# ubisoft/ubisoft-laforge-ZeroEGGS

Hardware: NVIDIA H100
Metric: frames/sec (train step, 60fps 75-joint pose) (higher is better)
Workload: dtype bf16

## Files before the change

ubisoft-laforge-zeroeggs_b200/csrc/decoder_bwd_tc.cu:

```cuda
#include "decoder_bwd_common.cuh"
#include "tc_dec_common.cuh"

namespace zeggs {

constexpr int BT_RING = 3;
constexpr int BT_XPART = 32768;
constexpr int BT_ACC_LD = 132;

struct BtGeom {
  int N2, N3, N4, P6;
  int kbH;
  int wslot;
  int slot_bytes;
  size_t off[4];
  size_t cta_bytes;
};

inline BtGeom make_btgeom(const DecGeom& g, const BwdGeom&) {
  BtGeom t;
  t.P6 = round_up(6 * g.U, 16); t.N2 = t.P6; t.N3 = t.P6 + 48; t.N4 = 16;
  t.kbH = ceil_div(g.H, 64);
  t.wslot = round_up(t.N3 * 128, 1024);
  t.slot_bytes = BT_XPART + 2 * t.wslot;
  size_t off = 0;
  t.off[0] = off; off += (size_t)t.kbH * t.N2 * 128;
  t.off[1] = off; off += (size_t)t.kbH * t.N3 * 128;
  t.off[2] = off; off += (size_t)t.kbH * t.N4 * 128;
  t.off[3] = off;
  t.cta_bytes = off;
  return t;
}

__global__ void pack_decoder_bwd_tc_kernel(DecGeom g, BtGeom tg, const float* __restrict__ Mfold, const float* __restrict__ W0,
                                           const float* __restrict__ Wih0, const float* __restrict__ Whh0,
                                           const float* __restrict__ Wih1, const float* __restrict__ Whh1, uint8_t* __restrict__ out) {
  const int H = g.H, U = g.U, A = g.A;
  const size_t per = tg.cta_bytes / 16, total = (size_t)g.G * per;
  for (size_t i = blockIdx.x * (size_t)blockDim.x + threadIdx.x; i < total; i += (size_t)gridDim.x * blockDim.x) {
    const int c = (int)(i / per);
    size_t ci = i % per;
    int chain = 2;
    for (int q = 0; q < 2; ++q) if (ci < tg.off[q + 1] / 16) { chain = q; break; }
    ci -= tg.off[chain] / 16;
    const int N = chain == 0 ? tg.N2 : chain == 1 ? tg.N3 : tg.N4;
    const int row = (int)(ci % N), cl = (int)((ci / N) % 8), kb = (int)(ci / ((size_t)8 * N));
    const int k0 = kb * 64 + cl * 8;
    const float* src = nullptr; size_t stride = 0;
    if (k0 < H) {
      if (chain <= 1 && row < 6 * U) {
        const int wsel = row / U, u = row % U, gq = wsel % 3, j = c * U + u;
        const size_t r = (size_t)(gq * H + k0);
        if (chain == 0) { src = (wsel < 3 ? Wih1 : Whh1) + r * H + j; stride = H; }
        else if (wsel < 3) { src = Wih0 + r * (A + H) + j; stride = A + H; }
        else { src = Whh0 + r * H + j; stride = H; }
      } else if (chain == 1 && row >= tg.P6) {
        const int rr = row - tg.P6, gq = rr / 16, lr = rr % 16;
        if (lr < U) { src = Mfold + ((size_t)(1 + gq) * H + k0) * H + c * U + lr; stride = H; }
        else if (lr >= 8 && lr < 11) { src = Wih0 + (size_t)(gq * H + k0) * (A + H) + H + P_OUT + (lr - 8); stride = A + H; }
      } else if (chain == 2) {
        if (row < U) { src = Mfold + (size_t)k0 * H + c * U + row; stride = H; }
        else if (row >= 8 && row < 11) { src = W0 + (size_t)k0 * A + P_OUT + (row - 8); stride = A; }
      }
    }
    __nv_bfloat16 t[8];
#pragma unroll
    for (int e = 0; e < 8; ++e) t[e] = __float2bfloat16_rn(src ? __ldg(src + (size_t)e * stride) : 0.f);
    uint8_t* dst = out + (size_t)c * tg.cta_bytes + tg.off[chain] + (size_t)kb * N * 128 + (size_t)row * 128 + (size_t)((cl ^ (row & 7)) << 4);
    *reinterpret_cast<uint4*>(dst) = *reinterpret_cast<const uint4*>(t);
  }
}

struct BtWs { uint8_t *g1img, *g0img, *dpaimg; const float* pre; float* dch; long long* dbg; size_t bytes; };
long long* tc_debug_buffer();
inline BtWs make_btws(void* base, const DecGeom& g) {
  BtWs w; size_t off = 0;
  auto take = [&](size_t n) { uint8_t* p = base ? (uint8_t*)base + off : nullptr; off += ((n + 1023) / 1024) * 1024; return p; };
  const size_t kbH = ceil_div(g.H, 64);
  w.g1img = take(kbH * 16384); w.g0img = take(kbH * 16384); w.dpaimg = take(kbH * 4096);
  w.pre = nullptr; w.dch = nullptr; w.dbg = nullptr;
  w.bytes = off; return w;
}

#define BTDBG1(ev) do { if (iw.dbg && c == 1 && lane == 0 && (T - 1 - t) < 64) iw.dbg[(T - 1 - t) * 32 + (ev)] = clock64(); } while (0)
#define BTDBG(ev) do { if (iw.dbg && c == 0 && lane == 0 && (T - 1 - t) < 64) iw.dbg[(T - 1 - t) * 32 + (ev)] = clock64(); } while (0)

template <int U>
__device__ __forceinline__ void store_img_row(uint8_t* img, int rows, int row, int j0, const float (&h)[U]) {
  __nv_bfloat16 t[U];
#pragma unroll
  for (int i = 0; i < U; ++i) t[i] = __float2bfloat16_rn(h[i]);
  uint8_t* p = img + img_off(rows, row, j0);
  if (U == 8) *reinterpret_cast<uint4*>(p) = *reinterpret_cast<const uint4*>(t);
  else *reinterpret_cast<uint2*>(p) = *reinterpret_cast<const uint2*>(t);
}

template <int U>
__global__ void __launch_bounds__(224, 1)
decoder_bwd_tc_kernel(zeggs_decoder_fwd_args a, DecGeom g, BwdGeom bg, BtGeom tg, DecWs w, BwdWs bw, BtWs iw, BwdArgsDev d,
                      const uint8_t* __restrict__ packed) {
  constexpr int P6 = (6 * U + 15) / 16 * 16, N2 = P6, N3 = P6 + 48, N4 = 16;
  constexpr int LD = BT_ACC_LD;
  extern __shared__ __align__(1024) uint8_t smem_raw[];
  uint8_t* smem = reinterpret_cast<uint8_t*>((reinterpret_cast<uintptr_t>(smem_raw) + 1023) & ~uintptr_t(1023));
  uint8_t* ring = smem;
  uint8_t* tail = ring + (size_t)BT_RING * tg.slot_bytes;
  uint64_t* full = reinterpret_cast<uint64_t*>(tail);
  uint64_t* empty = full + BT_RING;
  uint64_t* d_full = empty + BT_RING;
  float* accs = reinterpret_cast<float*>(tail + 512);
  float* c_w2r = accs + N3 * LD;
  float* c_gis = c_w2r + 6 * U;

  const int warp = __shfl_sync(0xffffffffu, (int)(threadIdx.x >> 5), 0), lane = threadIdx.x & 31;
  const int c = blockIdx.x, H = a.H, T = a.T;
  const int kbH = tg.kbH;
  const uint8_t* pk = packed + (size_t)c * tg.cta_bytes;
  constexpr int W_EPI = 4, W_PROD = 5, W_LOAD = 6;

  if (threadIdx.x == 0) {
    for (int i = 0; i < BT_RING; ++i) { mbar_init(&full[i], 2); mbar_init(&empty[i], 4); }
    for (int i = 0; i < 3; ++i) mbar_init(&d_full[i], 1);
    fence_mbar_init();
  }
  if (threadIdx.x < 6 * U) {
    const int n = threadIdx.x / U, u = threadIdx.x % U;
    c_w2r[threadIdx.x] = a.W2[(size_t)n * H + c * U + u] * a.out_std[n];
  }
  if (threadIdx.x < 3) c_gis[threadIdx.x] = 1.0f / a.in_std[P_OUT + threadIdx.x];
  __syncthreads();
  const size_t actH = (size_t)g.nbt * H * 32, act3 = (size_t)g.nbt * 3 * H * 32, act4 = (size_t)g.nbt * 4 * H * 32;

  if (warp == W_PROD) {
    if (lane == 0) {
      uint32_t it = 0;
      auto stream = [&](int chain, int nkb, int N, int kps) {
        const uint8_t* src = pk + tg.off[chain];
        const uint32_t tile = (uint32_t)N * 128;
        for (int kb = 0; kb < nkb; kb += kps, ++it) {
          const uint32_t s = it % BT_RING, ph = (it / BT_RING) & 1;
          const uint32_t bytes = (uint32_t)min(kps, nkb - kb) * tile;
          mbar_wait(&empty[s], ph ^ 1);
          mbar_arrive_expect_tx(&full[s], bytes);
          bulk_g2s(ring + (size_t)s * tg.slot_bytes + BT_XPART, src + (size_t)kb * tile, bytes, &full[s]);
        }
      };
      for (int t = T - 1; t >= 1; --t) {
        stream(0, kbH, tg.N2, 2); stream(1, kbH, tg.N3, 2);
        if (t > 1) stream(2, kbH, tg.N4, 8);
      }
    }
  } else if (warp == W_LOAD) {
    if (lane == 0) {
      uint32_t it = 0; unsigned epoch = 0;
      int t = T - 1; int sidx = 0;
      auto stream = [&](const uint8_t* img, int nkb, uint32_t tile_bytes) {
        grid_wait(bw.bar, (++epoch) * gridDim.x);
        if (iw.dbg && c == 0 && (T - 1 - t) < 64) iw.dbg[(T - 1 - t) * 32 + 2 * (sidx & 3)] = clock64();
        ++sidx;
        fence_proxy_async();
        const int kps = BT_XPART / (int)tile_bytes;
        for (int kb = 0; kb < nkb; kb += kps, ++it) {
          const uint32_t s = it % BT_RING, ph = (it / BT_RING) & 1;
          const uint32_t bytes = (uint32_t)min(kps, nkb - kb) * tile_bytes;
          mbar_wait(&empty[s], ph ^ 1);
          mbar_arrive_expect_tx(&full[s], bytes);
          bulk_g2s(ring + (size_t)s * tg.slot_bytes, img + (size_t)kb * tile_bytes, bytes, &full[s]);
        }
      };
      for (t = T - 1; t >= 1; --t) {
        sidx = 0;
        stream(iw.g1img, kbH, 16384); BTDBG(3);
        stream(iw.g0img, kbH, 16384); BTDBG(5);
        if (t > 1) { stream(iw.dpaimg, kbH, 4096); BTDBG(7); }
      }
    }
  } else if (warp < 4) {
    uint32_t it = 0;
    const uint64_t dR = make_smem_desc_sw128(ring);
    const uint32_t sstep = (uint32_t)(tg.slot_bytes >> 4);
    float d2[2][N2 / 2], d3[2][N3 / 2], d4[2][N4 / 2];
    auto chain_mma = [&](auto& dd, auto two, int nkb, int kps, uint32_t atile) {
      constexpr int N = 2 * (int)(sizeof(dd[0]) / sizeof(float));
      constexpr bool TWO = decltype(two)::value;
      const uint32_t astep = atile >> 4, wstep = (uint32_t)(N * 128) >> 4;
      uint32_t prev = 0;
      for (int kb = 0; kb < nkb; kb += kps, ++it) {
        const uint32_t s = it % BT_RING, ph = (it / BT_RING) & 1;
        const int nk = min(kps, nkb - kb);
        mbar_wait(&full[s], ph);
        uint64_t da = dR + (uint64_t)s * sstep, db = da + (BT_XPART >> 4);
        wgmma_fence();
        for (int kk = 0; kk < nk; ++kk, da += astep, db += wstep) {
#pragma unroll
          for (int ks = 0; ks < 4; ++ks) {
            const uint32_t acc = (kb + kk + ks) > 0 ? 1u : 0u;
            Wgmma<N>::mma(dd[0], da + 2 * ks, db + 2 * ks, acc);
            if constexpr (TWO) Wgmma<N>::mma(dd[1], da + 512 + 2 * ks, db + 2 * ks, acc);
          }
        }
        wgmma_commit();
        if (kb > 0) {
          wgmma_wait<1>();
          if (lane == 0) mbar_arrive(&empty[prev]);
        }
        prev = s;
      }
      wgmma_wait<0>();
      wgmma_fence_operands(dd[0]);
      if (TWO) wgmma_fence_operands(dd[1]);
      if (lane == 0) mbar_arrive(&empty[prev]);
      stage_acc<N>(dd[0], accs, LD, 0, TWO ? 64 : 32);
      if constexpr (TWO) stage_acc<N>(dd[1], accs, LD, 64, 64);
    };
    auto publish = [&](int i) {
      named_bar(1, 128);
      if (threadIdx.x == 0) mbar_arrive(&d_full[i]);
    };
    for (int t = T - 1; t >= 1; --t) {
      chain_mma(d2, std::true_type(), kbH, 2, 16384); publish(0); BTDBG(9);
      chain_mma(d3, std::true_type(), kbH, 2, 16384); publish(1); BTDBG(10);
      if (t > 1) { chain_mma(d4, std::false_type(), kbH, 8, 4096); publish(2); BTDBG(11); }
    }
  } else if (warp == W_EPI) {
    const int b = lane;
    const bool live = b < a.B;
    const int j0 = c * U;
    auto A = [&](int col, int blk) { return accs[(size_t)col * LD + 32 * blk + b]; };
    float dpq[7] = {0.f, 0.f, 0.f, 0.f, 0.f, 0.f, 0.f};
    float rpv[3] = {}, rqv[4] = {}, gpv[3] = {}, rq1v[4] = {}, ytv[6] = {}, e1p[3] = {}, e1q[4] = {}, e0p[3] = {}, e0q[4] = {};
    Q4 r_qinv, r_q1, r_E; V3 r_u, r_a1, r_a2, r_x; float r_k0 = 0.f, r_k1 = 0.f, r_k2 = 0.f;
    auto R_prefetch = [&](int t, bool have_dxp) {
      if (!live) return;
      const size_t bt = (size_t)b * T + t;
#pragma unroll
      for (int i = 0; i < 3; ++i) {
        rpv[i] = a.root_pos[bt * 3 + i];
        gpv[i] = have_dxp ? a.gaze_pos[(bt + 1) * 3 + i] : 0.f;
        e1p[i] = d.dRootPos ? d.dRootPos[(bt - 1) * 3 + i] : 0.f;
        e0p[i] = (!have_dxp && d.dRootPos) ? d.dRootPos[bt * 3 + i] : 0.f;
      }
#pragma unroll
      for (int i = 0; i < 4; ++i) {
        rqv[i] = a.root_rot[bt * 4 + i];
        rq1v[i] = a.root_rot[(bt - 1) * 4 + i];
        e1q[i] = d.dRootRot ? d.dRootRot[(bt - 1) * 4 + i] : 0.f;
        e0q[i] = (!have_dxp && d.dRootRot) ? d.dRootRot[bt * 4 + i] : 0.f;
      }
#pragma unroll
      for (int i = 0; i < 6; ++i) ytv[i] = a.Y[bt * P_OUT + i];
    };
    auto R_precompute = [&]() {
      if (!live) return;
      Q4 qt; qt.w = rqv[0]; qt.x = rqv[1]; qt.y = rqv[2]; qt.z = rqv[3];
      r_qinv = quat_inv(qt);
      r_u = v3(gpv[0] - rpv[0], gpv[1] - rpv[1], gpv[2] - rpv[2]);
      r_q1.w = rq1v[0]; r_q1.x = rq1v[1]; r_q1.y = rq1v[2]; r_q1.z = rq1v[3];
      r_a1 = a.dt * v3(ytv[0], ytv[1], ytv[2]);
      r_a2 = a.dt * v3(ytv[3], ytv[4], ytv[5]);
      const V3 wv = quat_mul_vec(r_q1, r_a2);
      r_E = quat_from_helical(wv);
      r_x = 0.5f * wv;
      const float a2 = dot(r_x, r_x), an = sqrtf(a2);
      if (an < 1e-5f) {
        const float rn = sqrtf(1.0f + a2), n = rn + 1e-5f;
        r_k0 = 1.0f / n; r_k1 = -1.0f / (n * n * rn); r_k2 = r_k1;
      } else {
        const float sn = sinf(an), cs = cosf(an);
        r_k0 = sn / an; r_k1 = -sn / an; r_k2 = (an * cs - sn) / (a2 * an);
      }
    };
    auto R_adjoint = [&](const float (&dgz)[3], bool have_dxp, float (&dch)[6]) {
#pragma unroll
      for (int i = 0; i < 6; ++i) dch[i] = 0.f;
      if (!live) return;
      V3 dp; Q4 dq;
      if (!have_dxp) {
        dp = v3(e0p[0], e0p[1], e0p[2]); dq.w = e0q[0]; dq.x = e0q[1]; dq.y = e0q[2]; dq.z = e0q[3];
      } else {
        dp = v3(dpq[0], dpq[1], dpq[2]); dq.w = dpq[3]; dq.x = dpq[4]; dq.y = dpq[5]; dq.z = dpq[6];
        Q4 dqc; V3 du;
        quat_mul_vec_bwd(r_qinv, r_u, v3(dgz[0], dgz[1], dgz[2]), dqc, du);
        dq.w += dqc.w; dq.x -= dqc.x; dq.y -= dqc.y; dq.z -= dqc.z;
        dp = dp - du;
      }
      Q4 dq_a, dq_b, dq_c, dE; V3 da1, da2;
      quat_mul_vec_bwd(r_q1, r_a1, dp, dq_a, da1);
      quat_mul_bwd(r_E, r_q1, dq, dE, dq_b);
      const V3 dEv = v3(dE.x, dE.y, dE.z);
      const V3 dw = 0.5f * (r_k0 * dEv + (r_k1 * dE.w + r_k2 * dot(dEv, r_x)) * r_x);
      quat_mul_vec_bwd(r_q1, r_a2, dw, dq_c, da2);
      dch[0] = a.dt * da1.x; dch[1] = a.dt * da1.y; dch[2] = a.dt * da1.z; dch[3] = a.dt * da2.x; dch[4] = a.dt * da2.y; dch[5] = a.dt * da2.z;
      dpq[0] = dp.x + e1p[0]; dpq[1] = dp.y + e1p[1]; dpq[2] = dp.z + e1p[2];
      dpq[3] = dq_a.w + dq_b.w + dq_c.w + e1q[0]; dpq[4] = dq_a.x + dq_b.x + dq_c.x + e1q[1];
      dpq[5] = dq_a.y + dq_b.y + dq_c.y + e1q[2]; dpq[6] = dq_a.z + dq_b.z + dq_c.z + e1q[3];
    };
    float dhz1[U], dhz0[U], dsum[16];
    float g1r[U], g1z[U], g1n[U], g1hn[U], g1hp[U], g1acc[U], prev[U];
    auto G1_prefetch = [&](int t) {
      const float* G = w.G1 + t * act4;
#pragma unroll
      for (int u = 0; u < U; ++u) {
        const int j = j0 + u;
        g1r[u] = G[(size_t)(0 * H + j) * 32 + b]; g1z[u] = G[(size_t)(1 * H + j) * 32 + b];
        g1n[u] = G[(size_t)(2 * H + j) * 32 + b]; g1hn[u] = G[(size_t)(3 * H + j) * 32 + b];
        g1hp[u] = w.H1[(t - 1) * actH + (size_t)j * 32 + b];
        g1acc[u] = t == T - 1 ? 0.f : bw.DH1[(size_t)j * 32 + b];
      }
      const float* P = iw.pre + ((size_t)(live ? b : 0) * T + t) * H + j0;
#pragma unroll
      for (int u4 = 0; u4 < U; u4 += 4) {
        const float4 v4 = live ? __ldg(reinterpret_cast<const float4*>(P + u4)) : make_float4(0.f, 0.f, 0.f, 0.f);
        prev[u4] = v4.x; prev[u4 + 1] = v4.y; prev[u4 + 2] = v4.z; prev[u4 + 3] = v4.w;
      }
    };
    auto G1_adjoint = [&](int t, const float (&fold)[U], const float (&dch)[6]) {
      float pr[U], pz[U], pn[U], pnr[U];
#pragma unroll
      for (int u = 0; u < U; ++u) {
        float dh = prev[u] + fold[u] + g1acc[u];
#pragma unroll
        for (int n = 0; n < 6; ++n) dh = fmaf(c_w2r[n * U + u], dch[n], dh);
        float dgi[3], dgh[3];
        gru_gate_bwd(dh, g1r[u], g1z[u], g1n[u], g1hn[u], g1hp[u], dgi, dgh, dhz1[u]);
        pr[u] = dgi[0]; pz[u] = dgi[1]; pn[u] = dgi[2]; pnr[u] = dgh[2];
      }
      store_img_row<U>(iw.g1img, 128, 0 * 32 + b, j0, pr); store_img_row<U>(iw.g1img, 128, 1 * 32 + b, j0, pz);
      store_img_row<U>(iw.g1img, 128, 2 * 32 + b, j0, pn); store_img_row<U>(iw.g1img, 128, 3 * 32 + b, j0, pnr);
      grid_arrive(bw.bar);
#pragma unroll
      for (int u = 0; u < U; ++u) {
        const int j = j0 + u;
        bw.DGI1[t * act3 + (size_t)(0 * H + j) * 32 + b] = pr[u]; bw.DGI1[t * act3 + (size_t)(1 * H + j) * 32 + b] = pz[u];
        bw.DGI1[t * act3 + (size_t)(2 * H + j) * 32 + b] = pn[u];
        bw.DGH1[t * act3 + (size_t)(0 * H + j) * 32 + b] = pr[u]; bw.DGH1[t * act3 + (size_t)(1 * H + j) * 32 + b] = pz[u];
        bw.DGH1[t * act3 + (size_t)(2 * H + j) * 32 + b] = pnr[u];
      }
      if (c == 0 && live) {
        float* dc = iw.dch + ((size_t)t * 32 + b) * 8;
#pragma unroll
        for (int n = 0; n < 6; ++n) dc[n] = dch[n];
      }
    };

    {
      const float zero3[3] = {0.f, 0.f, 0.f};
      float zeroU[U], dch[6];
#pragma unroll
      for (int u = 0; u < U; ++u) zeroU[u] = 0.f;
      R_prefetch(T - 1, false); R_precompute(); G1_prefetch(T - 1);
      R_adjoint(zero3, false, dch);
      G1_adjoint(T - 1, zeroU, dch);
    }
    for (int t = T - 1; t >= 1; --t) {
      const uint32_t ph = (uint32_t)((T - 1 - t) & 1);
      float gr[U], gz[U], gn[U], ghn[U], hp[U], acc[U];
      {
        const float* G = w.G0 + t * act4;
#pragma unroll
        for (int u = 0; u < U; ++u) {
          const int j = j0 + u;
          gr[u] = G[(size_t)(0 * H + j) * 32 + b]; gz[u] = G[(size_t)(1 * H + j) * 32 + b];
          gn[u] = G[(size_t)(2 * H + j) * 32 + b]; ghn[u] = G[(size_t)(3 * H + j) * 32 + b];
          hp[u] = w.H0[(t - 1) * actH + (size_t)j * 32 + b];
          acc[u] = t == T - 1 ? 0.f : bw.DH0[(size_t)j * 32 + b];
        }
      }
      mbar_wait(&d_full[0], ph);
      BTDBG(14);
      {
        float pr[U], pz[U], pn[U], pnr[U], dh1n[U];
#pragma unroll
        for (int u = 0; u < U; ++u) {
          const float oa = (A(0 * U + u, 0) + A(1 * U + u, 1)) + A(2 * U + u, 2);
          const float ob = (A(3 * U + u, 0) + A(4 * U + u, 1)) + A(5 * U + u, 3);
          float dgi[3], dgh[3];
          gru_gate_bwd(oa + acc[u], gr[u], gz[u], gn[u], ghn[u], hp[u], dgi, dgh, dhz0[u]);
          pr[u] = dgi[0]; pz[u] = dgi[1]; pn[u] = dgi[2]; pnr[u] = dgh[2];
          dh1n[u] = ob + dhz1[u];
        }
        store_img_row<U>(iw.g0img, 128, 0 * 32 + b, j0, pr); store_img_row<U>(iw.g0img, 128, 1 * 32 + b, j0, pz);
        store_img_row<U>(iw.g0img, 128, 2 * 32 + b, j0, pn); store_img_row<U>(iw.g0img, 128, 3 * 32 + b, j0, pnr);
        BTDBG(16);
        grid_arrive(bw.bar);
#pragma unroll
        for (int u = 0; u < U; ++u) bw.DH1[(size_t)(j0 + u) * 32 + b] = dh1n[u];
#pragma unroll
        for (int u = 0; u < U; ++u) {
          const int j = j0 + u;
          bw.DGI0[t * act3 + (size_t)(0 * H + j) * 32 + b] = pr[u]; bw.DGI0[t * act3 + (size_t)(1 * H + j) * 32 + b] = pz[u];
          bw.DGI0[t * act3 + (size_t)(2 * H + j) * 32 + b] = pn[u];
          bw.DGH0[t * act3 + (size_t)(0 * H + j) * 32 + b] = pr[u]; bw.DGH0[t * act3 + (size_t)(1 * H + j) * 32 + b] = pz[u];
          bw.DGH0[t * act3 + (size_t)(2 * H + j) * 32 + b] = pnr[u];
        }
      }
      float av[U];
#pragma unroll
      for (int u = 0; u < U; ++u) av[u] = w.A[t * actH + (size_t)(j0 + u) * 32 + b];
      mbar_wait(&d_full[1], ph);
      BTDBG(17);
      {
        float dpa[U], dh0n[U];
#pragma unroll
        for (int u = 0; u < U; ++u) {
          const float da = (A(0 * U + u, 0) + A(1 * U + u, 1)) + A(2 * U + u, 2);
          const float ob = (A(3 * U + u, 0) + A(4 * U + u, 1)) + A(5 * U + u, 3);
          dpa[u] = da * (av[u] > 0.f ? 1.f : av[u] + 1.f);
          dh0n[u] = ob + dhz0[u];
        }
#pragma unroll
        for (int r = 0; r < 16; ++r)
          dsum[r] = (A(P6 + r, 0) + A(P6 + 16 + r, 1)) + A(P6 + 32 + r, 2);
        store_img_row<U>(iw.dpaimg, 32, b, j0, dpa);
        BTDBG(18);
        if (t > 1) grid_arrive(bw.bar);
#pragma unroll
        for (int u = 0; u < U; ++u) { bw.DH0[(size_t)(j0 + u) * 32 + b] = dh0n[u]; bw.DPA[t * actH + (size_t)(j0 + u) * 32 + b] = dpa[u]; }
      }
      if (t == 1) break;
      R_prefetch(t - 1, true); R_precompute(); G1_prefetch(t - 1);
      mbar_wait(&d_full[2], ph);
      BTDBG(19);
      float tot[16];
#pragma unroll
      for (int r = 0; r < 16; ++r) tot[r] = A(r, 0) + dsum[r];
      float fold[U], dgz[3], dch[6];
#pragma unroll
      for (int u = 0; u < U; ++u) fold[u] = tot[u];
#pragma unroll
      for (int i = 0; i < 3; ++i) dgz[i] = tot[8 + i] * c_gis[i];
      R_adjoint(dgz, true, dch);
      BTDBG(20);
      G1_adjoint(t - 1, fold, dch);
    }
  }
}

__global__ void dy_scale_bf16_kernel(const float* __restrict__ dY, const float* __restrict__ os, size_t rows, int ld, __nv_bfloat16* __restrict__ out) {
  const size_t total = rows * (size_t)ld;
  for (size_t i = blockIdx.x * (size_t)blockDim.x + threadIdx.x; i < total; i += (size_t)gridDim.x * blockDim.x) {
    const size_t r = i / ld; const int n = (int)(i % ld);
    out[i] = __float2bfloat16_rn((dY && n < P_OUT) ? dY[r * P_OUT + n] * os[n] : 0.f);
  }
}

extern "C" size_t zeggs_decoder_packed_bwd_tc_bytes(int H, int S, int Z) {
  if (!tc_hidden_ok(H)) return 0;
  DecGeom g = make_geom(1, H, S, Z);
  BtGeom tg = make_btgeom(g, make_bgeom(g));
  return (size_t)g.G * tg.cta_bytes;
}
extern "C" size_t zeggs_decoder_bwd_tc_workspace_bytes(int H, int S, int Z) {
  if (!tc_hidden_ok(H)) return 0;
  return make_btws(nullptr, make_geom(1, H, S, Z)).bytes;
}
extern "C" int zeggs_decoder_pack_weights_bwd_tc(const zeggs_decoder_fwd_args* a, void* packed, void* stream_) {
  CtxScope ctx_scope(a ? a->ctx : nullptr);
  ZCHECK_ARG(a && packed, "decoder bwd tc pack: bad arguments");
  ZCHECK_SUPPORTED(tc_hidden_ok(a->H), "decoder bwd tc pack: hidden size %d unsupported (needs H %% 128 == 0, 384 <= H <= 1024)", a->H);
  const float* mfold = decoder_tc_mfold(*a);
  ZCHECK_ARG(mfold != nullptr, "decoder bwd tc pack: the forward pack (zeggs_decoder_pack_weights_tc -> args.packed_tc) must run first");
  DecGeom g = make_geom(a->B, a->H, a->S, a->Z);
  BwdGeom bg = make_bgeom(g);
  BtGeom tg = make_btgeom(g, bg);
  ZCHECK_ARG(g.U <= 8, "decoder bwd tc: unsupported units per CTA");
  ScopedTimer tm_pack("weight_pack", (cudaStream_t)stream_);
  pack_decoder_bwd_tc_kernel<<<592, 256, 0, (cudaStream_t)stream_>>>(g, tg, mfold, a->W0, a->W_ih0, a->W_hh0, a->W_ih1, a->W_hh1, (uint8_t*)packed);
  count_launch();
  ZCHECK_LAUNCH();
  return ZEGGS_OK;
}

template <int U>
static int launch_bt(const zeggs_decoder_fwd_args& a, const DecGeom& g, const BwdGeom& bg, const BtGeom& tg, const DecWs& w,
                     const BwdWs& bw, const BtWs& iw, const BwdArgsDev& d, const uint8_t* packed, cudaStream_t stream) {
  const size_t smem = 1024 + (size_t)BT_RING * tg.slot_bytes + 512 + (size_t)(tg.N3 * BT_ACC_LD + 6 * U + 16) * sizeof(float);
  static size_t checked_smem = 0;
  if (checked_smem != smem) {
    ZCHECK_CUDA(cudaFuncSetAttribute(decoder_bwd_tc_kernel<U>, cudaFuncAttributeMaxDynamicSharedMemorySize, (int)smem));
    int dev = 0, nsm = 0, occ = 0;
    ZCHECK_CUDA(cudaGetDevice(&dev));
    ZCHECK_CUDA(cudaDeviceGetAttribute(&nsm, cudaDevAttrMultiProcessorCount, dev));
    ZCHECK_CUDA(cudaOccupancyMaxActiveBlocksPerMultiprocessor(&occ, decoder_bwd_tc_kernel<U>, 224, smem));
    ZCHECK_ARG(occ * nsm >= g.G, "decoder bwd tc: cooperative grid of %d CTAs does not fit", g.G);
    checked_smem = smem;
  }
  void* args[] = {(void*)&a, (void*)&g, (void*)&bg, (void*)&tg, (void*)&w, (void*)&bw, (void*)&iw, (void*)&d, (void*)&packed};
  ZCHECK_CUDA(cudaLaunchCooperativeKernel((void*)decoder_bwd_tc_kernel<U>, dim3(g.G), dim3(224), args, smem, stream));
  count_launch();
  return ZEGGS_OK;
}

int decoder_bwd_tc_run(const zeggs_decoder_fwd_args& a, const zeggs_decoder_bwd_args& b, const DecGeom& g, const DecWs& w,
                       const BwdWs& bw, cudaStream_t stream) {
  BwdGeom bg = make_bgeom(g);
  ZCHECK_ARG(g.nbt == 1, "decoder bwd tc engine needs B <= 32 (got B=%d)", a.B);
  ZCHECK_ARG(b.packed_bwd_tc && b.workspace_tc, "decoder bwd tc: packed_bwd_tc / workspace_tc missing");
  BtGeom tg = make_btgeom(g, bg);
  ZCHECK_ARG((tg.kbH % 2) == 0, "decoder bwd tc: unsupported geometry");
  BtWs iw = make_btws(b.workspace_tc, g);
  iw.dbg = tc_debug_buffer();
  iw.dch = bw.DCH;
  const int H = a.H, ld = round_up(P_OUT, 8);
  const size_t rows = (size_t)a.B * a.T;
  char* p = scratch_base();
  ZCHECK_ARG(p != nullptr, "decoder bwd tc: scratch buffer missing (zeggs_ctx.scratch)");
  auto take = [&](size_t bytes) { char* r = p; p += (bytes + 255) / 256 * 256; return r; };
  __nv_bfloat16* dys = (__nv_bfloat16*)take(rows * ld * 2);
  __nv_bfloat16* w2t = (__nv_bfloat16*)take((size_t)H * ld * 2);
  float* pre = (float*)take(rows * H * sizeof(float));
  ZCHECK_ARG((size_t)(p - scratch_base()) <= scratch_bytes(), "decoder bwd tc: scratch buffer too small (%zu bytes needed)", (size_t)(p - scratch_base()));
  dy_scale_bf16_kernel<<<1184, 256, 0, stream>>>(b.dY, a.out_std, rows, ld, dys); count_launch();
  int rc = split_t_launch(a.W2, P_OUT, H, H, w2t, nullptr, ld, stream); if (rc) return rc;
  rc = tc_gemm_launch((int)rows, H, ld, dys, nullptr, ld, w2t, nullptr, ld, nullptr, pre, H, 0, 0, stream); if (rc) return rc;
  iw.pre = pre;
  BwdArgsDev d; d.dY = b.dY; d.dRootPos = b.dRootPos; d.dRootRot = b.dRootRot; d.packed = nullptr;
  return g.U == 4 ? launch_bt<4>(a, g, bg, tg, w, bw, iw, d, (const uint8_t*)b.packed_bwd_tc, stream)
                  : launch_bt<8>(a, g, bg, tg, w, bw, iw, d, (const uint8_t*)b.packed_bwd_tc, stream);
}

}
```

ubisoft-laforge-zeroeggs_b200/csrc/tc_common.cuh:

```cuda
#pragma once
#include <cuda.h>
#include <cuda_runtime.h>
#include <stdint.h>
#include <type_traits>

namespace zeggs {

__device__ __forceinline__ uint32_t smem_u32(const void* p) { return (uint32_t)__cvta_generic_to_shared(p); }

__device__ __forceinline__ void mbar_init(uint64_t* bar, uint32_t count) {
  asm volatile("mbarrier.init.shared::cta.b64 [%0], %1;\n" ::"r"(smem_u32(bar)), "r"(count) : "memory");
}
__device__ __forceinline__ void fence_mbar_init() {
  asm volatile("fence.mbarrier_init.release.cluster;\n" ::: "memory");
  asm volatile("fence.proxy.async.shared::cta;\n" ::: "memory");
}
__device__ __forceinline__ void mbar_arrive_expect_tx(uint64_t* bar, uint32_t bytes) {
  asm volatile("mbarrier.arrive.expect_tx.shared::cta.b64 _, [%0], %1;\n" ::"r"(smem_u32(bar)), "r"(bytes) : "memory");
}
__device__ __forceinline__ void mbar_arrive(uint64_t* bar) {
  asm volatile("mbarrier.arrive.shared::cta.b64 _, [%0];\n" ::"r"(smem_u32(bar)) : "memory");
}
__device__ __forceinline__ void mbar_wait(uint64_t* bar, uint32_t parity) {
  const uint32_t addr = smem_u32(bar);
  uint32_t done = 0;
#pragma unroll 1
  for (uint32_t it = 0; it < 20000000u; ++it) {
    asm volatile("{\n .reg .pred p;\n mbarrier.try_wait.parity.shared::cta.b64 p, [%1], %2;\n selp.u32 %0, 1, 0, p;\n}\n"
                 : "=r"(done) : "r"(addr), "r"(parity) : "memory");
    if (done) return;
  }
  __trap();
}

__device__ __forceinline__ bool elect_one_sync() {
  uint32_t pred;
  asm volatile("{\n .reg .pred p;\n elect.sync _|p, 0xffffffff;\n selp.u32 %0, 1, 0, p;\n}\n" : "=r"(pred));
  return pred != 0;
}

__device__ __forceinline__ void tma_prefetch_desc(const CUtensorMap* m) {
  asm volatile("prefetch.tensormap [%0];\n" ::"l"(reinterpret_cast<uint64_t>(m)) : "memory");
}
__device__ __forceinline__ void tma_load_2d(void* smem_dst, const CUtensorMap* m, uint64_t* bar, int c0, int c1) {
  asm volatile("cp.async.bulk.tensor.2d.shared::cluster.global.mbarrier::complete_tx::bytes [%0], [%1, {%3, %4}], [%2];\n"
               ::"r"(smem_u32(smem_dst)), "l"(reinterpret_cast<uint64_t>(m)), "r"(smem_u32(bar)), "r"(c0), "r"(c1) : "memory");
}
__device__ __forceinline__ void tma_load_3d(void* smem_dst, const CUtensorMap* m, uint64_t* bar, int c0, int c1, int c2) {
  asm volatile("cp.async.bulk.tensor.3d.shared::cluster.global.mbarrier::complete_tx::bytes [%0], [%1, {%3, %4, %5}], [%2];\n"
               ::"r"(smem_u32(smem_dst)), "l"(reinterpret_cast<uint64_t>(m)), "r"(smem_u32(bar)), "r"(c0), "r"(c1), "r"(c2) : "memory");
}

__device__ __forceinline__ void wgmma_fence() { asm volatile("wgmma.fence.sync.aligned;\n" ::: "memory"); }
__device__ __forceinline__ void wgmma_commit() { asm volatile("wgmma.commit_group.sync.aligned;\n" ::: "memory"); }
template <int n>
__device__ __forceinline__ void wgmma_wait() { asm volatile("wgmma.wait_group.sync.aligned %0;\n" ::"n"(n) : "memory"); }
template <int R>
__device__ __forceinline__ void wgmma_fence_operands(float (&d)[R]) {
#pragma unroll
  for (int i = 0; i < R; ++i) asm volatile("" : "+f"(d[i])::"memory");
}
__device__ __forceinline__ void named_bar(int id, int nthreads) { asm volatile("bar.sync %0, %1;\n" ::"r"(id), "r"(nthreads) : "memory"); }

template <int N> struct Wgmma;
template <> struct Wgmma<16> {
  static __device__ __forceinline__ void mma(float (&d)[8], uint64_t a, uint64_t b, uint32_t scale_d) {
    asm volatile("{\n .reg .pred p;\n setp.ne.b32 p, %10, 0;\n"
                 "wgmma.mma_async.sync.aligned.m64n16k16.f32.bf16.bf16 {%0, %1, %2, %3, %4, %5, %6, %7}, %8, %9, p, 1, 1, 0, 0;\n}\n"
                 : "+f"(d[0]), "+f"(d[1]), "+f"(d[2]), "+f"(d[3]), "+f"(d[4]), "+f"(d[5]), "+f"(d[6]), "+f"(d[7])
                 : "l"(a), "l"(b), "r"(scale_d));
  }
};
template <> struct Wgmma<24> {
  static __device__ __forceinline__ void mma(float (&d)[12], uint64_t a, uint64_t b, uint32_t scale_d) {
    asm volatile("{\n .reg .pred p;\n setp.ne.b32 p, %14, 0;\n"
                 "wgmma.mma_async.sync.aligned.m64n24k16.f32.bf16.bf16 {%0, %1, %2, %3, %4, %5, %6, %7, %8, %9, %10, %11}, %12, %13, p, 1, 1, 0, 0;\n}\n"
                 : "+f"(d[0]), "+f"(d[1]), "+f"(d[2]), "+f"(d[3]), "+f"(d[4]), "+f"(d[5]), "+f"(d[6]), "+f"(d[7]), "+f"(d[8]), "+f"(d[9]), "+f"(d[10]), "+f"(d[11])
                 : "l"(a), "l"(b), "r"(scale_d));
  }
};
template <> struct Wgmma<32> {
  static __device__ __forceinline__ void mma(float (&d)[16], uint64_t a, uint64_t b, uint32_t scale_d) {
    asm volatile("{\n .reg .pred p;\n setp.ne.b32 p, %18, 0;\n"
                 "wgmma.mma_async.sync.aligned.m64n32k16.f32.bf16.bf16 {%0, %1, %2, %3, %4, %5, %6, %7, %8, %9, %10, %11, %12, %13, %14, %15}, %16, %17, p, 1, 1, 0, 0;\n}\n"
                 : "+f"(d[0]), "+f"(d[1]), "+f"(d[2]), "+f"(d[3]), "+f"(d[4]), "+f"(d[5]), "+f"(d[6]), "+f"(d[7]), "+f"(d[8]), "+f"(d[9]), "+f"(d[10]), "+f"(d[11]), "+f"(d[12]), "+f"(d[13]), "+f"(d[14]), "+f"(d[15])
                 : "l"(a), "l"(b), "r"(scale_d));
  }
};
template <> struct Wgmma<40> {
  static __device__ __forceinline__ void mma(float (&d)[20], uint64_t a, uint64_t b, uint32_t scale_d) {
    asm volatile("{\n .reg .pred p;\n setp.ne.b32 p, %22, 0;\n"
                 "wgmma.mma_async.sync.aligned.m64n40k16.f32.bf16.bf16 {%0, %1, %2, %3, %4, %5, %6, %7, %8, %9, %10, %11, %12, %13, %14, %15, %16, %17, %18, %19}, %20, %21, p, 1, 1, 0, 0;\n}\n"
                 : "+f"(d[0]), "+f"(d[1]), "+f"(d[2]), "+f"(d[3]), "+f"(d[4]), "+f"(d[5]), "+f"(d[6]), "+f"(d[7]), "+f"(d[8]), "+f"(d[9]), "+f"(d[10]), "+f"(d[11]), "+f"(d[12]), "+f"(d[13]), "+f"(d[14]), "+f"(d[15]), "+f"(d[16]), "+f"(d[17]), "+f"(d[18]), "+f"(d[19])
                 : "l"(a), "l"(b), "r"(scale_d));
  }
};
template <> struct Wgmma<48> {
  static __device__ __forceinline__ void mma(float (&d)[24], uint64_t a, uint64_t b, uint32_t scale_d) {
    asm volatile("{\n .reg .pred p;\n setp.ne.b32 p, %26, 0;\n"
                 "wgmma.mma_async.sync.aligned.m64n48k16.f32.bf16.bf16 {%0, %1, %2, %3, %4, %5, %6, %7, %8, %9, %10, %11, %12, %13, %14, %15, %16, %17, %18, %19, %20, %21, %22, %23}, %24, %25, p, 1, 1, 0, 0;\n}\n"
                 : "+f"(d[0]), "+f"(d[1]), "+f"(d[2]), "+f"(d[3]), "+f"(d[4]), "+f"(d[5]), "+f"(d[6]), "+f"(d[7]), "+f"(d[8]), "+f"(d[9]), "+f"(d[10]), "+f"(d[11]), "+f"(d[12]), "+f"(d[13]), "+f"(d[14]), "+f"(d[15]), "+f"(d[16]), "+f"(d[17]), "+f"(d[18]), "+f"(d[19]), "+f"(d[20]), "+f"(d[21]), "+f"(d[22]), "+f"(d[23])
                 : "l"(a), "l"(b), "r"(scale_d));
  }
};
template <> struct Wgmma<80> {
  static __device__ __forceinline__ void mma(float (&d)[40], uint64_t a, uint64_t b, uint32_t scale_d) {
    asm volatile("{\n .reg .pred p;\n setp.ne.b32 p, %42, 0;\n"
                 "wgmma.mma_async.sync.aligned.m64n80k16.f32.bf16.bf16 {%0, %1, %2, %3, %4, %5, %6, %7, %8, %9, %10, %11, %12, %13, %14, %15, %16, %17, %18, %19, %20, %21, %22, %23, %24, %25, %26, %27, %28, %29, %30, %31, %32, %33, %34, %35, %36, %37, %38, %39}, %40, %41, p, 1, 1, 0, 0;\n}\n"
                 : "+f"(d[0]), "+f"(d[1]), "+f"(d[2]), "+f"(d[3]), "+f"(d[4]), "+f"(d[5]), "+f"(d[6]), "+f"(d[7]), "+f"(d[8]), "+f"(d[9]), "+f"(d[10]), "+f"(d[11]), "+f"(d[12]), "+f"(d[13]), "+f"(d[14]), "+f"(d[15]), "+f"(d[16]), "+f"(d[17]), "+f"(d[18]), "+f"(d[19]), "+f"(d[20]), "+f"(d[21]), "+f"(d[22]), "+f"(d[23]), "+f"(d[24]), "+f"(d[25]), "+f"(d[26]), "+f"(d[27]), "+f"(d[28]), "+f"(d[29]), "+f"(d[30]), "+f"(d[31]), "+f"(d[32]), "+f"(d[33]), "+f"(d[34]), "+f"(d[35]), "+f"(d[36]), "+f"(d[37]), "+f"(d[38]), "+f"(d[39])
                 : "l"(a), "l"(b), "r"(scale_d));
  }
};
template <> struct Wgmma<96> {
  static __device__ __forceinline__ void mma(float (&d)[48], uint64_t a, uint64_t b, uint32_t scale_d) {
    asm volatile("{\n .reg .pred p;\n setp.ne.b32 p, %50, 0;\n"
                 "wgmma.mma_async.sync.aligned.m64n96k16.f32.bf16.bf16 {%0, %1, %2, %3, %4, %5, %6, %7, %8, %9, %10, %11, %12, %13, %14, %15, %16, %17, %18, %19, %20, %21, %22, %23, %24, %25, %26, %27, %28, %29, %30, %31, %32, %33, %34, %35, %36, %37, %38, %39, %40, %41, %42, %43, %44, %45, %46, %47}, %48, %49, p, 1, 1, 0, 0;\n}\n"
                 : "+f"(d[0]), "+f"(d[1]), "+f"(d[2]), "+f"(d[3]), "+f"(d[4]), "+f"(d[5]), "+f"(d[6]), "+f"(d[7]), "+f"(d[8]), "+f"(d[9]), "+f"(d[10]), "+f"(d[11]), "+f"(d[12]), "+f"(d[13]), "+f"(d[14]), "+f"(d[15]), "+f"(d[16]), "+f"(d[17]), "+f"(d[18]), "+f"(d[19]), "+f"(d[20]), "+f"(d[21]), "+f"(d[22]), "+f"(d[23]), "+f"(d[24]), "+f"(d[25]), "+f"(d[26]), "+f"(d[27]), "+f"(d[28]), "+f"(d[29]), "+f"(d[30]), "+f"(d[31]), "+f"(d[32]), "+f"(d[33]), "+f"(d[34]), "+f"(d[35]), "+f"(d[36]), "+f"(d[37]), "+f"(d[38]), "+f"(d[39]), "+f"(d[40]), "+f"(d[41]), "+f"(d[42]), "+f"(d[43]), "+f"(d[44]), "+f"(d[45]), "+f"(d[46]), "+f"(d[47])
                 : "l"(a), "l"(b), "r"(scale_d));
  }
};
template <> struct Wgmma<128> {
  static __device__ __forceinline__ void mma(float (&d)[64], uint64_t a, uint64_t b, uint32_t scale_d) {
    asm volatile("{\n .reg .pred p;\n setp.ne.b32 p, %66, 0;\n"
                 "wgmma.mma_async.sync.aligned.m64n128k16.f32.bf16.bf16 {%0, %1, %2, %3, %4, %5, %6, %7, %8, %9, %10, %11, %12, %13, %14, %15, %16, %17, %18, %19, %20, %21, %22, %23, %24, %25, %26, %27, %28, %29, %30, %31, %32, %33, %34, %35, %36, %37, %38, %39, %40, %41, %42, %43, %44, %45, %46, %47, %48, %49, %50, %51, %52, %53, %54, %55, %56, %57, %58, %59, %60, %61, %62, %63}, %64, %65, p, 1, 1, 0, 0;\n}\n"
                 : "+f"(d[0]), "+f"(d[1]), "+f"(d[2]), "+f"(d[3]), "+f"(d[4]), "+f"(d[5]), "+f"(d[6]), "+f"(d[7]), "+f"(d[8]), "+f"(d[9]), "+f"(d[10]), "+f"(d[11]), "+f"(d[12]), "+f"(d[13]), "+f"(d[14]), "+f"(d[15]), "+f"(d[16]), "+f"(d[17]), "+f"(d[18]), "+f"(d[19]), "+f"(d[20]), "+f"(d[21]), "+f"(d[22]), "+f"(d[23]), "+f"(d[24]), "+f"(d[25]), "+f"(d[26]), "+f"(d[27]), "+f"(d[28]), "+f"(d[29]), "+f"(d[30]), "+f"(d[31]), "+f"(d[32]), "+f"(d[33]), "+f"(d[34]), "+f"(d[35]), "+f"(d[36]), "+f"(d[37]), "+f"(d[38]), "+f"(d[39]), "+f"(d[40]), "+f"(d[41]), "+f"(d[42]), "+f"(d[43]), "+f"(d[44]), "+f"(d[45]), "+f"(d[46]), "+f"(d[47]), "+f"(d[48]), "+f"(d[49]), "+f"(d[50]), "+f"(d[51]), "+f"(d[52]), "+f"(d[53]), "+f"(d[54]), "+f"(d[55]), "+f"(d[56]), "+f"(d[57]), "+f"(d[58]), "+f"(d[59]), "+f"(d[60]), "+f"(d[61]), "+f"(d[62]), "+f"(d[63])
                 : "l"(a), "l"(b), "r"(scale_d));
  }
};

__device__ __forceinline__ uint64_t make_smem_desc_sw128(const void* tile) {
  const uint32_t addr = smem_u32(tile);
  uint64_t d = 0;
  d |= (uint64_t)((addr & 0x3FFFFu) >> 4);
  d |= (uint64_t)1 << 16;
  d |= (uint64_t)(1024 >> 4) << 32;
  d |= (uint64_t)1 << 62;
  return d;
}

typedef CUresult (*PFN_encodeTiled)(CUtensorMap*, CUtensorMapDataType, cuuint32_t, void*, const cuuint64_t*,
                                    const cuuint64_t*, const cuuint32_t*, const cuuint32_t*, CUtensorMapInterleave,
                                    CUtensorMapSwizzle, CUtensorMapL2promotion, CUtensorMapFloatOOBfill);
inline PFN_encodeTiled get_encode_fn() {
  static PFN_encodeTiled fn = nullptr;
  if (!fn) {
    void* p = nullptr;
    cudaDriverEntryPointQueryResult q;
    if (cudaGetDriverEntryPoint("cuTensorMapEncodeTiled", &p, cudaEnableDefault, &q) == cudaSuccess &&
        q == cudaDriverEntryPointSuccess)
      fn = (PFN_encodeTiled)p;
  }
  return fn;
}

}
```

ubisoft-laforge-zeroeggs_b200/csrc/tc_dec_common.cuh:

```cuda
#pragma once
#include "decoder_common.cuh"
#include "tc_common.cuh"

namespace zeggs {

__host__ __device__ inline size_t img_off(int rows, int row, int k) {
  const int kb = k >> 6, c = (k & 63) >> 3, e = k & 7;
  return (size_t)kb * rows * 128 + (size_t)row * 128 + (size_t)((c ^ (row & 7)) << 4) + (size_t)e * 2;
}


__device__ __forceinline__ void bulk_g2s(void* smem_dst, const void* gsrc, uint32_t bytes, uint64_t* bar) {
  asm volatile("cp.async.bulk.shared::cluster.global.mbarrier::complete_tx::bytes [%0], [%1], %2, [%3];\n"
               ::"r"(smem_u32(smem_dst)), "l"(gsrc), "r"(bytes), "r"(smem_u32(bar)) : "memory");
}

__device__ __forceinline__ uint32_t cluster_ctarank() { uint32_t r; asm volatile("mov.u32 %0, %%cluster_ctarank;\n" : "=r"(r)); return r; }
__device__ __forceinline__ uint32_t cluster_nctarank() { uint32_t r; asm volatile("mov.u32 %0, %%cluster_nctarank;\n" : "=r"(r)); return r; }
__device__ __forceinline__ void cluster_sync_all() {
  asm volatile("barrier.cluster.arrive.release.aligned;\n" ::: "memory");
  asm volatile("barrier.cluster.wait.acquire.aligned;\n" ::: "memory");
}
__device__ __forceinline__ void bulk_g2s_multicast(void* smem_dst, const void* gsrc, uint32_t bytes, uint64_t* bar, uint16_t mask) {
  asm volatile("cp.async.bulk.shared::cluster.global.mbarrier::complete_tx::bytes.multicast::cluster [%0], [%1], %2, [%3], %4;\n"
               ::"r"(smem_u32(smem_dst)), "l"(gsrc), "r"(bytes), "r"(smem_u32(bar)), "h"(mask) : "memory");
}
__device__ __forceinline__ void fence_proxy_async() { asm volatile("fence.proxy.async;\n" ::: "memory"); }

template <int N>
__device__ __forceinline__ void stage_acc(const float (&d)[N / 2], float* out, int ld, int row0, int nrows) {
  const int wq = (threadIdx.x >> 5) & 3, lane = threadIdx.x & 31;
  const int r = 16 * wq + (lane >> 2), c = 2 * (lane & 3);
#pragma unroll
  for (int i = 0; i < N / 8; ++i) {
    if (r < nrows) { out[(size_t)(8 * i + c) * ld + row0 + r] = d[4 * i]; out[(size_t)(8 * i + c + 1) * ld + row0 + r] = d[4 * i + 1]; }
    if (r + 8 < nrows) { out[(size_t)(8 * i + c) * ld + row0 + r + 8] = d[4 * i + 2]; out[(size_t)(8 * i + c + 1) * ld + row0 + r + 8] = d[4 * i + 3]; }
  }
}
template <int NC>
__device__ __forceinline__ void acc_ld(const float* p, int ld, float (&v)[NC]) {
#pragma unroll
  for (int i = 0; i < NC; ++i) v[i] = p[(size_t)i * ld];
}

__device__ __forceinline__ float fast_sigmoid(float x) { return __fdividef(1.0f, 1.0f + __expf(-x)); }
__device__ __forceinline__ float fast_tanh(float x) { return 1.0f - __fdividef(2.0f, 1.0f + __expf(2.0f * x)); }

__device__ __forceinline__ void grid_arrive(unsigned* counter) {
  __syncwarp();
  if ((threadIdx.x & 31) == 0) asm volatile("red.release.gpu.global.add.u32 [%0], 1;\n" ::"l"(counter) : "memory");
}
__device__ __forceinline__ void grid_wait(const unsigned* counter, unsigned target) {
  long long t0 = clock64();
  while (ld_acquire_u32(counter) < target) {
    if (clock64() - t0 > 4000000000LL) __trap();
  }
}

template <int U>
__device__ __forceinline__ void store_img_units(uint8_t* img, int b, int j0, const float (&h)[U]) {
  __nv_bfloat16 t[U];
#pragma unroll
  for (int i = 0; i < U; ++i) t[i] = __float2bfloat16_rn(h[i]);
  uint8_t* p = img + img_off(32, b, j0);
  if (U == 8) *reinterpret_cast<uint4*>(p) = *reinterpret_cast<const uint4*>(t);
  else *reinterpret_cast<uint2*>(p) = *reinterpret_cast<const uint2*>(t);
}


}
```

Measured before the change: 501,600.

## Split decoder backward GEMMs across CTA pairs using 2-CTA clusters and DSMEM reduction

Launches the backward decoder kernel in clusters of two CTAs. Each CTA loads half of the activation-gradient image along the batch-row dimension (8 KB parts instead of the full 16 KB tile) and runs single 64-row wgmmas over a 2U-unit weight tile that is shared by the pair. The epilogue then reads and sums partial accumulators from both CTAs' shared memory through distributed shared memory, with cross-CTA mbarrier signalling. The aim is to halve the MMA and transfer work per CTA on the serial recurrent critical path. In exchange it adds cluster-scope synchronization and remote shared-memory loads in the epilogue, and it repacks the weights and reorders the gate rows.

Result: faster. 534,100 (median of 6 runs) (+6.5%).

```diff
diff --git a/ubisoft-laforge-zeroeggs_b200/csrc/decoder_bwd_tc.cu b/ubisoft-laforge-zeroeggs_b200/csrc/decoder_bwd_tc.cu
--- a/ubisoft-laforge-zeroeggs_b200/csrc/decoder_bwd_tc.cu
+++ b/ubisoft-laforge-zeroeggs_b200/csrc/decoder_bwd_tc.cu
@@ -3,60 +3,61 @@
 
 namespace zeggs {
 
-constexpr int BT_RING = 3;
-constexpr int BT_XPART = 32768;
-constexpr int BT_ACC_LD = 132;
+constexpr int BT_RING = 4;
+constexpr int BT_XPART = 16384;
+constexpr int BT_ACC_LD = 68;
 
 struct BtGeom {
-  int N2, N3, N4, P6;
+  int N2, N3[2], N4, FG;
   int kbH;
   int wslot;
   int slot_bytes;
-  size_t off[4];
+  size_t off[3];
   size_t cta_bytes;
 };
 
 inline BtGeom make_btgeom(const DecGeom& g, const BwdGeom&) {
   BtGeom t;
-  t.P6 = round_up(6 * g.U, 16); t.N2 = t.P6; t.N3 = t.P6 + 48; t.N4 = 16;
+  t.FG = round_up(2 * g.U + 3, 8);
+  t.N2 = 6 * g.U; t.N3[0] = t.N2 + t.FG; t.N3[1] = t.N2 + 2 * t.FG; t.N4 = 16;
   t.kbH = ceil_div(g.H, 64);
-  t.wslot = round_up(t.N3 * 128, 1024);
+  t.wslot = round_up(t.N3[1] * 128, 1024);
   t.slot_bytes = BT_XPART + 2 * t.wslot;
-  size_t off = 0;
-  t.off[0] = off; off += (size_t)t.kbH * t.N2 * 128;
-  t.off[1] = off; off += (size_t)t.kbH * t.N3 * 128;
-  t.off[2] = off; off += (size_t)t.kbH * t.N4 * 128;
-  t.off[3] = off;
-  t.cta_bytes = off;
+  t.off[0] = 0;
+  t.off[2] = (size_t)t.kbH * t.N2 * 128;
+  t.off[1] = t.off[2] + (size_t)t.kbH * t.N4 * 128;
+  t.cta_bytes = t.off[1] + (size_t)t.kbH * t.N3[1] * 128;
   return t;
 }
 
 __global__ void pack_decoder_bwd_tc_kernel(DecGeom g, BtGeom tg, const float* __restrict__ Mfold, const float* __restrict__ W0,
                                            const float* __restrict__ Wih0, const float* __restrict__ Whh0,
                                            const float* __restrict__ Wih1, const float* __restrict__ Whh1, uint8_t* __restrict__ out) {
-  const int H = g.H, U = g.U, A = g.A;
+  const int H = g.H, U = g.U, A = g.A, N2 = tg.N2, FG = tg.FG;
   const size_t per = tg.cta_bytes / 16, total = (size_t)g.G * per;
   for (size_t i = blockIdx.x * (size_t)blockDim.x + threadIdx.x; i < total; i += (size_t)gridDim.x * blockDim.x) {
-    const int c = (int)(i / per);
+    const int c = (int)(i / per), rk = c & 1, p = c >> 1;
     size_t ci = i % per;
-    int chain = 2;
-    for (int q = 0; q < 2; ++q) if (ci < tg.off[q + 1] / 16) { chain = q; break; }
+    const int chain = ci < tg.off[2] / 16 ? 0 : ci < tg.off[1] / 16 ? 2 : 1;
     ci -= tg.off[chain] / 16;
-    const int N = chain == 0 ? tg.N2 : chain == 1 ? tg.N3 : tg.N4;
+    const int N = chain == 0 ? N2 : chain == 1 ? tg.N3[rk] : tg.N4;
+    if (ci >= (size_t)tg.kbH * 8 * N) continue;
     const int row = (int)(ci % N), cl = (int)((ci / N) % 8), kb = (int)(ci / ((size_t)8 * N));
     const int k0 = kb * 64 + cl * 8;
     const float* src = nullptr; size_t stride = 0;
     if (k0 < H) {
-      if (chain <= 1 && row < 6 * U) {
-        const int wsel = row / U, u = row % U, gq = wsel % 3, j = c * U + u;
+      if (chain <= 1 && row < N2) {
+        const int grp = row / (2 * U), j = p * 2 * U + row % (2 * U);
+        const bool ih = rk == 0 ? grp == 0 : grp != 1;
+        const int gq = grp == 2 ? 2 : rk;
         const size_t r = (size_t)(gq * H + k0);
-        if (chain == 0) { src = (wsel < 3 ? Wih1 : Whh1) + r * H + j; stride = H; }
-        else if (wsel < 3) { src = Wih0 + r * (A + H) + j; stride = A + H; }
+        if (chain == 0) { src = (ih ? Wih1 : Whh1) + r * H + j; stride = H; }
+        else if (ih) { src = Wih0 + r * (A + H) + j; stride = A + H; }
         else { src = Whh0 + r * H + j; stride = H; }
-      } else if (chain == 1 && row >= tg.P6) {
-        const int rr = row - tg.P6, gq = rr / 16, lr = rr % 16;
-        if (lr < U) { src = Mfold + ((size_t)(1 + gq) * H + k0) * H + c * U + lr; stride = H; }
-        else if (lr >= 8 && lr < 11) { src = Wih0 + (size_t)(gq * H + k0) * (A + H) + H + P_OUT + (lr - 8); stride = A + H; }
+      } else if (chain == 1) {
+        const int f = (row - N2) / FG, lr = (row - N2) % FG, gq = rk + f;
+        if (lr < 2 * U) { src = Mfold + ((size_t)(1 + gq) * H + k0) * H + p * 2 * U + lr; stride = H; }
+        else if (lr < 2 * U + 3) { src = Wih0 + (size_t)(gq * H + k0) * (A + H) + H + P_OUT + (lr - 2 * U); stride = A + H; }
       } else if (chain == 2) {
         if (row < U) { src = Mfold + (size_t)k0 * H + c * U + row; stride = H; }
         else if (row >= 8 && row < 11) { src = W0 + (size_t)k0 * A + P_OUT + (row - 8); stride = A; }
@@ -81,8 +82,7 @@
   w.bytes = off; return w;
 }
 
-#define BTDBG1(ev) do { if (iw.dbg && c == 1 && lane == 0 && (T - 1 - t) < 64) iw.dbg[(T - 1 - t) * 32 + (ev)] = clock64(); } while (0)
-#define BTDBG(ev) do { if (iw.dbg && c == 0 && lane == 0 && (T - 1 - t) < 64) iw.dbg[(T - 1 - t) * 32 + (ev)] = clock64(); } while (0)
+#define BTDBG(ev) do { if (iw.dbg && c < 2 && lane == 0 && (T - 1 - t) < 64) iw.dbg[c * 2048 + (T - 1 - t) * 32 + (ev)] = clock64(); } while (0)
 
 template <int U>
 __device__ __forceinline__ void store_img_row(uint8_t* img, int rows, int row, int j0, const float (&h)[U]) {
@@ -98,7 +98,7 @@
 __global__ void __launch_bounds__(224, 1)
 decoder_bwd_tc_kernel(zeggs_decoder_fwd_args a, DecGeom g, BwdGeom bg, BtGeom tg, DecWs w, BwdWs bw, BtWs iw, BwdArgsDev d,
                       const uint8_t* __restrict__ packed) {
-  constexpr int P6 = (6 * U + 15) / 16 * 16, N2 = P6, N3 = P6 + 48, N4 = 16;
+  constexpr int N2 = 6 * U, FG = (2 * U + 3 + 7) / 8 * 8, N3A = N2 + FG, N3B = N2 + 2 * FG, N4 = 16;
   constexpr int LD = BT_ACC_LD;
   extern __shared__ __align__(1024) uint8_t smem_raw[];
   uint8_t* smem = reinterpret_cast<uint8_t*>((reinterpret_cast<uintptr_t>(smem_raw) + 1023) & ~uintptr_t(1023));
@@ -107,19 +107,22 @@
   uint64_t* full = reinterpret_cast<uint64_t*>(tail);
   uint64_t* empty = full + BT_RING;
   uint64_t* d_full = empty + BT_RING;
-  float* accs = reinterpret_cast<float*>(tail + 512);
-  float* c_w2r = accs + N3 * LD;
+  float* acc2 = reinterpret_cast<float*>(tail + 512);
+  float* acc3 = acc2 + N2 * LD;
+  float* acc4 = acc3 + N3B * LD;
+  float* c_w2r = acc4 + N4 * LD;
   float* c_gis = c_w2r + 6 * U;
 
   const int warp = __shfl_sync(0xffffffffu, (int)(threadIdx.x >> 5), 0), lane = threadIdx.x & 31;
   const int c = blockIdx.x, H = a.H, T = a.T;
+  const int rk = c & 1, peer = rk ^ 1;
   const int kbH = tg.kbH;
   const uint8_t* pk = packed + (size_t)c * tg.cta_bytes;
   constexpr int W_EPI = 4, W_PROD = 5, W_LOAD = 6;
 
   if (threadIdx.x == 0) {
     for (int i = 0; i < BT_RING; ++i) { mbar_init(&full[i], 2); mbar_init(&empty[i], 4); }
-    for (int i = 0; i < 3; ++i) mbar_init(&d_full[i], 1);
+    mbar_init(&d_full[0], 2); mbar_init(&d_full[1], 2); mbar_init(&d_full[2], 1);
     fence_mbar_init();
   }
   if (threadIdx.x < 6 * U) {
@@ -127,7 +130,7 @@
     c_w2r[threadIdx.x] = a.W2[(size_t)n * H + c * U + u] * a.out_std[n];
   }
   if (threadIdx.x < 3) c_gis[threadIdx.x] = 1.0f / a.in_std[P_OUT + threadIdx.x];
-  __syncthreads();
+  cluster_sync_all();
   const size_t actH = (size_t)g.nbt * H * 32, act3 = (size_t)g.nbt * 3 * H * 32, act4 = (size_t)g.nbt * 4 * H * 32;
 
   if (warp == W_PROD) {
@@ -145,43 +148,44 @@
         }
       };
       for (int t = T - 1; t >= 1; --t) {
-        stream(0, kbH, tg.N2, 2); stream(1, kbH, tg.N3, 2);
-        if (t > 1) stream(2, kbH, tg.N4, 8);
+        stream(0, kbH, tg.N2, 2); stream(1, kbH, tg.N3[rk], 2);
+        if (t > 1) stream(2, kbH, tg.N4, 4);
       }
     }
   } else if (warp == W_LOAD) {
     if (lane == 0) {
       uint32_t it = 0; unsigned epoch = 0;
       int t = T - 1; int sidx = 0;
-      auto stream = [&](const uint8_t* img, int nkb, uint32_t tile_bytes) {
+      auto stream = [&](const uint8_t* img, int nkb, uint32_t tile_bytes, uint32_t part_bytes, uint32_t part_off) {
         grid_wait(bw.bar, (++epoch) * gridDim.x);
-        if (iw.dbg && c == 0 && (T - 1 - t) < 64) iw.dbg[(T - 1 - t) * 32 + 2 * (sidx & 3)] = clock64();
+        if (iw.dbg && c < 2 && (T - 1 - t) < 64) iw.dbg[c * 2048 + (T - 1 - t) * 32 + 2 * (sidx & 3)] = clock64();
         ++sidx;
         fence_proxy_async();
-        const int kps = BT_XPART / (int)tile_bytes;
+        const int kps = BT_XPART / (int)part_bytes;
         for (int kb = 0; kb < nkb; kb += kps, ++it) {
           const uint32_t s = it % BT_RING, ph = (it / BT_RING) & 1;
-          const uint32_t bytes = (uint32_t)min(kps, nkb - kb) * tile_bytes;
+          const int nk = min(kps, nkb - kb);
           mbar_wait(&empty[s], ph ^ 1);
-          mbar_arrive_expect_tx(&full[s], bytes);
-          bulk_g2s(ring + (size_t)s * tg.slot_bytes, img + (size_t)kb * tile_bytes, bytes, &full[s]);
+          mbar_arrive_expect_tx(&full[s], (uint32_t)nk * part_bytes);
+          for (int kk = 0; kk < nk; ++kk)
+            bulk_g2s(ring + (size_t)s * tg.slot_bytes + (size_t)kk * part_bytes, img + (size_t)(kb + kk) * tile_bytes + part_off,
+                     part_bytes, &full[s]);
         }
       };
       for (t = T - 1; t >= 1; --t) {
         sidx = 0;
-        stream(iw.g1img, kbH, 16384); BTDBG(3);
-        stream(iw.g0img, kbH, 16384); BTDBG(5);
-        if (t > 1) { stream(iw.dpaimg, kbH, 4096); BTDBG(7); }
+        stream(iw.g1img, kbH, 16384, 8192, rk * 8192); BTDBG(3);
+        stream(iw.g0img, kbH, 16384, 8192, rk * 8192); BTDBG(5);
+        if (t > 1) { stream(iw.dpaimg, kbH, 4096, 4096, 0); BTDBG(7); }
       }
     }
   } else if (warp < 4) {
     uint32_t it = 0;
     const uint64_t dR = make_smem_desc_sw128(ring);
     const uint32_t sstep = (uint32_t)(tg.slot_bytes >> 4);
-    float d2[2][N2 / 2], d3[2][N3 / 2], d4[2][N4 / 2];
-    auto chain_mma = [&](auto& dd, auto two, int nkb, int kps, uint32_t atile) {
-      constexpr int N = 2 * (int)(sizeof(dd[0]) / sizeof(float));
-      constexpr bool TWO = decltype(two)::value;
+    float d2[N2 / 2], d3a[N3A / 2], d3b[N3B / 2], d4[N4 / 2];
+    auto chain_mma = [&](auto& dd, int nkb, int kps, uint32_t atile, float* out, int nrows) {
+      constexpr int N = 2 * (int)(sizeof(dd) / sizeof(float));
       const uint32_t astep = atile >> 4, wstep = (uint32_t)(N * 128) >> 4;
       uint32_t prev = 0;
       for (int kb = 0; kb < nkb; kb += kps, ++it) {
@@ -192,11 +196,7 @@
         wgmma_fence();
         for (int kk = 0; kk < nk; ++kk, da += astep, db += wstep) {
 #pragma unroll
-          for (int ks = 0; ks < 4; ++ks) {
-            const uint32_t acc = (kb + kk + ks) > 0 ? 1u : 0u;
-            Wgmma<N>::mma(dd[0], da + 2 * ks, db + 2 * ks, acc);
-            if constexpr (TWO) Wgmma<N>::mma(dd[1], da + 512 + 2 * ks, db + 2 * ks, acc);
-          }
+          for (int ks = 0; ks < 4; ++ks) Wgmma<N>::mma(dd, da + 2 * ks, db + 2 * ks, (kb + kk + ks) > 0 ? 1u : 0u);
         }
         wgmma_commit();
         if (kb > 0) {
@@ -206,26 +206,31 @@
         prev = s;
       }
       wgmma_wait<0>();
-      wgmma_fence_operands(dd[0]);
-      if (TWO) wgmma_fence_operands(dd[1]);
+      wgmma_fence_operands(dd);
       if (lane == 0) mbar_arrive(&empty[prev]);
-      stage_acc<N>(dd[0], accs, LD, 0, TWO ? 64 : 32);
-      if constexpr (TWO) stage_acc<N>(dd[1], accs, LD, 64, 64);
+      stage_acc<N>(dd, out, LD, 0, nrows);
     };
     auto publish = [&](int i) {
       named_bar(1, 128);
-      if (threadIdx.x == 0) mbar_arrive(&d_full[i]);
+      if (threadIdx.x == 0) {
+        mbar_arrive(&d_full[i]);
+        if (i < 2) mbar_arrive_cluster(&d_full[i], (uint32_t)peer);
+      }
     };
     for (int t = T - 1; t >= 1; --t) {
-      chain_mma(d2, std::true_type(), kbH, 2, 16384); publish(0); BTDBG(9);
-      chain_mma(d3, std::true_type(), kbH, 2, 16384); publish(1); BTDBG(10);
-      if (t > 1) { chain_mma(d4, std::false_type(), kbH, 8, 4096); publish(2); BTDBG(11); }
+      chain_mma(d2, kbH, 2, 8192, acc2, 64); publish(0); BTDBG(9);
+      if (rk == 0) chain_mma(d3a, kbH, 2, 8192, acc3, 64);
+      else chain_mma(d3b, kbH, 2, 8192, acc3, 64);
+      publish(1); BTDBG(10);
+      if (t > 1) { chain_mma(d4, kbH, 4, 4096, acc4, 32); publish(2); BTDBG(11); }
     }
   } else if (warp == W_EPI) {
     const int b = lane;
     const bool live = b < a.B;
-    const int j0 = c * U;
-    auto A = [&](int col, int blk) { return accs[(size_t)col * LD + 32 * blk + b]; };
+    const int j0 = c * U, wo = rk * U;
+    const uint32_t a2r0 = cluster_map(acc2, 0u), a2r1 = cluster_map(acc2, 1u);
+    auto X = [&](uint32_t s, int col, int blk) { return ld_cluster_f32(s + (uint32_t)(col * LD + 32 * blk + b) * 4u); };
+    auto A = [&](const float* s, int col, int blk) { return s[(size_t)col * LD + 32 * blk + b]; };
     float dpq[7] = {0.f, 0.f, 0.f, 0.f, 0.f, 0.f, 0.f};
     float rpv[3] = {}, rqv[4] = {}, gpv[3] = {}, rq1v[4] = {}, ytv[6] = {}, e1p[3] = {}, e1q[4] = {}, e0p[3] = {}, e0q[4] = {};
     Q4 r_qinv, r_q1, r_E; V3 r_u, r_a1, r_a2, r_x; float r_k0 = 0.f, r_k1 = 0.f, r_k2 = 0.f;
@@ -294,7 +299,7 @@
       dpq[3] = dq_a.w + dq_b.w + dq_c.w + e1q[0]; dpq[4] = dq_a.x + dq_b.x + dq_c.x + e1q[1];
       dpq[5] = dq_a.y + dq_b.y + dq_c.y + e1q[2]; dpq[6] = dq_a.z + dq_b.z + dq_c.z + e1q[3];
     };
-    float dhz1[U], dhz0[U], dsum[16];
+    float dhz1[U], dhz0[U], dsf[U], dsg[3];
     float g1r[U], g1z[U], g1n[U], g1hn[U], g1hp[U], g1acc[U], prev[U];
     auto G1_prefetch = [&](int t) {
       const float* G = w.G1 + t * act4;
@@ -324,8 +329,8 @@
         gru_gate_bwd(dh, g1r[u], g1z[u], g1n[u], g1hn[u], g1hp[u], dgi, dgh, dhz1[u]);
         pr[u] = dgi[0]; pz[u] = dgi[1]; pn[u] = dgi[2]; pnr[u] = dgh[2];
       }
-      store_img_row<U>(iw.g1img, 128, 0 * 32 + b, j0, pr); store_img_row<U>(iw.g1img, 128, 1 * 32 + b, j0, pz);
-      store_img_row<U>(iw.g1img, 128, 2 * 32 + b, j0, pn); store_img_row<U>(iw.g1img, 128, 3 * 32 + b, j0, pnr);
+      store_img_row<U>(iw.g1img, 128, 0 * 32 + b, j0, pr); store_img_row<U>(iw.g1img, 128, 1 * 32 + b, j0, pnr);
+      store_img_row<U>(iw.g1img, 128, 2 * 32 + b, j0, pz); store_img_row<U>(iw.g1img, 128, 3 * 32 + b, j0, pn);
       grid_arrive(bw.bar);
 #pragma unroll
       for (int u = 0; u < U; ++u) {
@@ -365,21 +370,21 @@
           acc[u] = t == T - 1 ? 0.f : bw.DH0[(size_t)j * 32 + b];
         }
       }
-      mbar_wait(&d_full[0], ph);
+      mbar_wait_cluster(&d_full[0], ph);
       BTDBG(14);
       {
         float pr[U], pz[U], pn[U], pnr[U], dh1n[U];
 #pragma unroll
         for (int u = 0; u < U; ++u) {
-          const float oa = (A(0 * U + u, 0) + A(1 * U + u, 1)) + A(2 * U + u, 2);
-          const float ob = (A(3 * U + u, 0) + A(4 * U + u, 1)) + A(5 * U + u, 3);
+          const float oa = (X(a2r0, 0 * 2 * U + wo + u, 0) + X(a2r1, 0 * 2 * U + wo + u, 0)) + X(a2r1, 2 * 2 * U + wo + u, 1);
+          const float ob = (X(a2r0, 1 * 2 * U + wo + u, 0) + X(a2r1, 1 * 2 * U + wo + u, 0)) + X(a2r0, 2 * 2 * U + wo + u, 1);
           float dgi[3], dgh[3];
           gru_gate_bwd(oa + acc[u], gr[u], gz[u], gn[u], ghn[u], hp[u], dgi, dgh, dhz0[u]);
           pr[u] = dgi[0]; pz[u] = dgi[1]; pn[u] = dgi[2]; pnr[u] = dgh[2];
           dh1n[u] = ob + dhz1[u];
         }
-        store_img_row<U>(iw.g0img, 128, 0 * 32 + b, j0, pr); store_img_row<U>(iw.g0img, 128, 1 * 32 + b, j0, pz);
-        store_img_row<U>(iw.g0img, 128, 2 * 32 + b, j0, pn); store_img_row<U>(iw.g0img, 128, 3 * 32 + b, j0, pnr);
+        store_img_row<U>(iw.g0img, 128, 0 * 32 + b, j0, pr); store_img_row<U>(iw.g0img, 128, 1 * 32 + b, j0, pnr);
+        store_img_row<U>(iw.g0img, 128, 2 * 32 + b, j0, pz); store_img_row<U>(iw.g0img, 128, 3 * 32 + b, j0, pn);
         BTDBG(16);
         grid_arrive(bw.bar);
 #pragma unroll
@@ -396,20 +401,22 @@
       float av[U];
 #pragma unroll
       for (int u = 0; u < U; ++u) av[u] = w.A[t * actH + (size_t)(j0 + u) * 32 + b];
-      mbar_wait(&d_full[1], ph);
+      mbar_wait_cluster(&d_full[1], ph);
       BTDBG(17);
       {
         float dpa[U], dh0n[U];
 #pragma unroll
         for (int u = 0; u < U; ++u) {
-          const float da = (A(0 * U + u, 0) + A(1 * U + u, 1)) + A(2 * U + u, 2);
-          const float ob = (A(3 * U + u, 0) + A(4 * U + u, 1)) + A(5 * U + u, 3);
+          const float da = (X(a2r0, N2 + 0 * 2 * U + wo + u, 0) + X(a2r1, N2 + 0 * 2 * U + wo + u, 0)) + X(a2r1, N2 + 2 * 2 * U + wo + u, 1);
+          const float ob = (X(a2r0, N2 + 1 * 2 * U + wo + u, 0) + X(a2r1, N2 + 1 * 2 * U + wo + u, 0)) + X(a2r0, N2 + 2 * 2 * U + wo + u, 1);
           dpa[u] = da * (av[u] > 0.f ? 1.f : av[u] + 1.f);
           dh0n[u] = ob + dhz0[u];
         }
 #pragma unroll
-        for (int r = 0; r < 16; ++r)
-          dsum[r] = (A(P6 + r, 0) + A(P6 + 16 + r, 1)) + A(P6 + 32 + r, 2);
+        for (int u = 0; u < U; ++u) dsf[u] = (X(a2r0, N2 + N2 + wo + u, 0) + X(a2r1, N2 + N2 + wo + u, 0)) + X(a2r1, N2 + N2 + FG + wo + u, 1);
+#pragma unroll
+        for (int i = 0; i < 3; ++i)
+          dsg[i] = (X(a2r0, N2 + N2 + 2 * U + i, 0) + X(a2r1, N2 + N2 + 2 * U + i, 0)) + X(a2r1, N2 + N2 + FG + 2 * U + i, 1);
         store_img_row<U>(iw.dpaimg, 32, b, j0, dpa);
         BTDBG(18);
         if (t > 1) grid_arrive(bw.bar);
@@ -420,19 +427,17 @@
       R_prefetch(t - 1, true); R_precompute(); G1_prefetch(t - 1);
       mbar_wait(&d_full[2], ph);
       BTDBG(19);
-      float tot[16];
-#pragma unroll
-      for (int r = 0; r < 16; ++r) tot[r] = A(r, 0) + dsum[r];
       float fold[U], dgz[3], dch[6];
 #pragma unroll
-      for (int u = 0; u < U; ++u) fold[u] = tot[u];
-#pragma unroll
-      for (int i = 0; i < 3; ++i) dgz[i] = tot[8 + i] * c_gis[i];
+      for (int u = 0; u < U; ++u) fold[u] = A(acc4, u, 0) + dsf[u];
+#pragma unroll
+      for (int i = 0; i < 3; ++i) dgz[i] = (A(acc4, 8 + i, 0) + dsg[i]) * c_gis[i];
       R_adjoint(dgz, true, dch);
       BTDBG(20);
       G1_adjoint(t - 1, fold, dch);
     }
   }
+  cluster_sync_all();
 }
 
 __global__ void dy_scale_bf16_kernel(const float* __restrict__ dY, const float* __restrict__ os, size_t rows, int ld, __nv_bfloat16* __restrict__ out) {
@@ -473,19 +478,28 @@
 template <int U>
 static int launch_bt(const zeggs_decoder_fwd_args& a, const DecGeom& g, const BwdGeom& bg, const BtGeom& tg, const DecWs& w,
                      const BwdWs& bw, const BtWs& iw, const BwdArgsDev& d, const uint8_t* packed, cudaStream_t stream) {
-  const size_t smem = 1024 + (size_t)BT_RING * tg.slot_bytes + 512 + (size_t)(tg.N3 * BT_ACC_LD + 6 * U + 16) * sizeof(float);
+  const size_t smem = 1024 + (size_t)BT_RING * tg.slot_bytes + 512 +
+                      (size_t)((tg.N2 + tg.N3[1] + tg.N4) * BT_ACC_LD + 6 * U + 16) * sizeof(float);
+  cudaLaunchAttribute attr[2];
+  attr[0].id = cudaLaunchAttributeClusterDimension;
+  attr[0].val.clusterDim.x = 2; attr[0].val.clusterDim.y = 1; attr[0].val.clusterDim.z = 1;
+  attr[1].id = cudaLaunchAttributeCooperative;
+  attr[1].val.cooperative = 1;
+  cudaLaunchConfig_t cfg = {};
+  cfg.gridDim = dim3(g.G); cfg.blockDim = dim3(224); cfg.dynamicSmemBytes = smem; cfg.stream = stream;
+  cfg.attrs = attr; cfg.numAttrs = 2;
   static size_t checked_smem = 0;
+  static int max_clusters = 0;
   if (checked_smem != smem) {
     ZCHECK_CUDA(cudaFuncSetAttribute(decoder_bwd_tc_kernel<U>, cudaFuncAttributeMaxDynamicSharedMemorySize, (int)smem));
-    int dev = 0, nsm = 0, occ = 0;
-    ZCHECK_CUDA(cudaGetDevice(&dev));
-    ZCHECK_CUDA(cudaDeviceGetAttribute(&nsm, cudaDevAttrMultiProcessorCount, dev));
-    ZCHECK_CUDA(cudaOccupancyMaxActiveBlocksPerMultiprocessor(&occ, decoder_bwd_tc_kernel<U>, 224, smem));
-    ZCHECK_ARG(occ * nsm >= g.G, "decoder bwd tc: cooperative grid of %d CTAs does not fit", g.G);
+    cudaLaunchConfig_t occ = cfg;
+    occ.numAttrs = 1;
+    ZCHECK_CUDA(cudaOccupancyMaxActiveClusters(&max_clusters, decoder_bwd_tc_kernel<U>, &occ));
     checked_smem = smem;
   }
-  void* args[] = {(void*)&a, (void*)&g, (void*)&bg, (void*)&tg, (void*)&w, (void*)&bw, (void*)&iw, (void*)&d, (void*)&packed};
-  ZCHECK_CUDA(cudaLaunchCooperativeKernel((void*)decoder_bwd_tc_kernel<U>, dim3(g.G), dim3(224), args, smem, stream));
+  ZCHECK_ARG(2 * max_clusters >= g.G, "decoder bwd tc: cooperative grid of %d CTAs in clusters of 2 does not fit (%d clusters resident)",
+             g.G, max_clusters);
+  ZCHECK_CUDA(cudaLaunchKernelEx(&cfg, decoder_bwd_tc_kernel<U>, a, g, bg, tg, w, bw, iw, d, packed));
   count_launch();
   return ZEGGS_OK;
 }
diff --git a/ubisoft-laforge-zeroeggs_b200/csrc/tc_common.cuh b/ubisoft-laforge-zeroeggs_b200/csrc/tc_common.cuh
--- a/ubisoft-laforge-zeroeggs_b200/csrc/tc_common.cuh
+++ b/ubisoft-laforge-zeroeggs_b200/csrc/tc_common.cuh
@@ -79,14 +79,6 @@
                  : "l"(a), "l"(b), "r"(scale_d));
   }
 };
-template <> struct Wgmma<32> {
-  static __device__ __forceinline__ void mma(float (&d)[16], uint64_t a, uint64_t b, uint32_t scale_d) {
-    asm volatile("{\n .reg .pred p;\n setp.ne.b32 p, %18, 0;\n"
-                 "wgmma.mma_async.sync.aligned.m64n32k16.f32.bf16.bf16 {%0, %1, %2, %3, %4, %5, %6, %7, %8, %9, %10, %11, %12, %13, %14, %15}, %16, %17, p, 1, 1, 0, 0;\n}\n"
-                 : "+f"(d[0]), "+f"(d[1]), "+f"(d[2]), "+f"(d[3]), "+f"(d[4]), "+f"(d[5]), "+f"(d[6]), "+f"(d[7]), "+f"(d[8]), "+f"(d[9]), "+f"(d[10]), "+f"(d[11]), "+f"(d[12]), "+f"(d[13]), "+f"(d[14]), "+f"(d[15])
-                 : "l"(a), "l"(b), "r"(scale_d));
-  }
-};
 template <> struct Wgmma<40> {
   static __device__ __forceinline__ void mma(float (&d)[20], uint64_t a, uint64_t b, uint32_t scale_d) {
     asm volatile("{\n .reg .pred p;\n setp.ne.b32 p, %22, 0;\n"
@@ -103,11 +95,19 @@
                  : "l"(a), "l"(b), "r"(scale_d));
   }
 };
-template <> struct Wgmma<80> {
-  static __device__ __forceinline__ void mma(float (&d)[40], uint64_t a, uint64_t b, uint32_t scale_d) {
-    asm volatile("{\n .reg .pred p;\n setp.ne.b32 p, %42, 0;\n"
-                 "wgmma.mma_async.sync.aligned.m64n80k16.f32.bf16.bf16 {%0, %1, %2, %3, %4, %5, %6, %7, %8, %9, %10, %11, %12, %13, %14, %15, %16, %17, %18, %19, %20, %21, %22, %23, %24, %25, %26, %27, %28, %29, %30, %31, %32, %33, %34, %35, %36, %37, %38, %39}, %40, %41, p, 1, 1, 0, 0;\n}\n"
-                 : "+f"(d[0]), "+f"(d[1]), "+f"(d[2]), "+f"(d[3]), "+f"(d[4]), "+f"(d[5]), "+f"(d[6]), "+f"(d[7]), "+f"(d[8]), "+f"(d[9]), "+f"(d[10]), "+f"(d[11]), "+f"(d[12]), "+f"(d[13]), "+f"(d[14]), "+f"(d[15]), "+f"(d[16]), "+f"(d[17]), "+f"(d[18]), "+f"(d[19]), "+f"(d[20]), "+f"(d[21]), "+f"(d[22]), "+f"(d[23]), "+f"(d[24]), "+f"(d[25]), "+f"(d[26]), "+f"(d[27]), "+f"(d[28]), "+f"(d[29]), "+f"(d[30]), "+f"(d[31]), "+f"(d[32]), "+f"(d[33]), "+f"(d[34]), "+f"(d[35]), "+f"(d[36]), "+f"(d[37]), "+f"(d[38]), "+f"(d[39])
+template <> struct Wgmma<56> {
+  static __device__ __forceinline__ void mma(float (&d)[28], uint64_t a, uint64_t b, uint32_t scale_d) {
+    asm volatile("{\n .reg .pred p;\n setp.ne.b32 p, %30, 0;\n"
+                 "wgmma.mma_async.sync.aligned.m64n56k16.f32.bf16.bf16 {%0, %1, %2, %3, %4, %5, %6, %7, %8, %9, %10, %11, %12, %13, %14, %15, %16, %17, %18, %19, %20, %21, %22, %23, %24, %25, %26, %27}, %28, %29, p, 1, 1, 0, 0;\n}\n"
+                 : "+f"(d[0]), "+f"(d[1]), "+f"(d[2]), "+f"(d[3]), "+f"(d[4]), "+f"(d[5]), "+f"(d[6]), "+f"(d[7]), "+f"(d[8]), "+f"(d[9]), "+f"(d[10]), "+f"(d[11]), "+f"(d[12]), "+f"(d[13]), "+f"(d[14]), "+f"(d[15]), "+f"(d[16]), "+f"(d[17]), "+f"(d[18]), "+f"(d[19]), "+f"(d[20]), "+f"(d[21]), "+f"(d[22]), "+f"(d[23]), "+f"(d[24]), "+f"(d[25]), "+f"(d[26]), "+f"(d[27])
+                 : "l"(a), "l"(b), "r"(scale_d));
+  }
+};
+template <> struct Wgmma<72> {
+  static __device__ __forceinline__ void mma(float (&d)[36], uint64_t a, uint64_t b, uint32_t scale_d) {
+    asm volatile("{\n .reg .pred p;\n setp.ne.b32 p, %38, 0;\n"
+                 "wgmma.mma_async.sync.aligned.m64n72k16.f32.bf16.bf16 {%0, %1, %2, %3, %4, %5, %6, %7, %8, %9, %10, %11, %12, %13, %14, %15, %16, %17, %18, %19, %20, %21, %22, %23, %24, %25, %26, %27, %28, %29, %30, %31, %32, %33, %34, %35}, %36, %37, p, 1, 1, 0, 0;\n}\n"
+                 : "+f"(d[0]), "+f"(d[1]), "+f"(d[2]), "+f"(d[3]), "+f"(d[4]), "+f"(d[5]), "+f"(d[6]), "+f"(d[7]), "+f"(d[8]), "+f"(d[9]), "+f"(d[10]), "+f"(d[11]), "+f"(d[12]), "+f"(d[13]), "+f"(d[14]), "+f"(d[15]), "+f"(d[16]), "+f"(d[17]), "+f"(d[18]), "+f"(d[19]), "+f"(d[20]), "+f"(d[21]), "+f"(d[22]), "+f"(d[23]), "+f"(d[24]), "+f"(d[25]), "+f"(d[26]), "+f"(d[27]), "+f"(d[28]), "+f"(d[29]), "+f"(d[30]), "+f"(d[31]), "+f"(d[32]), "+f"(d[33]), "+f"(d[34]), "+f"(d[35])
                  : "l"(a), "l"(b), "r"(scale_d));
   }
 };
diff --git a/ubisoft-laforge-zeroeggs_b200/csrc/tc_dec_common.cuh b/ubisoft-laforge-zeroeggs_b200/csrc/tc_dec_common.cuh
--- a/ubisoft-laforge-zeroeggs_b200/csrc/tc_dec_common.cuh
+++ b/ubisoft-laforge-zeroeggs_b200/csrc/tc_dec_common.cuh
@@ -15,15 +15,33 @@
                ::"r"(smem_u32(smem_dst)), "l"(gsrc), "r"(bytes), "r"(smem_u32(bar)) : "memory");
 }
 
-__device__ __forceinline__ uint32_t cluster_ctarank() { uint32_t r; asm volatile("mov.u32 %0, %%cluster_ctarank;\n" : "=r"(r)); return r; }
-__device__ __forceinline__ uint32_t cluster_nctarank() { uint32_t r; asm volatile("mov.u32 %0, %%cluster_nctarank;\n" : "=r"(r)); return r; }
 __device__ __forceinline__ void cluster_sync_all() {
-  asm volatile("barrier.cluster.arrive.release.aligned;\n" ::: "memory");
-  asm volatile("barrier.cluster.wait.acquire.aligned;\n" ::: "memory");
+  asm volatile("barrier.cluster.arrive.release;\n" ::: "memory");
+  asm volatile("barrier.cluster.wait.acquire;\n" ::: "memory");
 }
-__device__ __forceinline__ void bulk_g2s_multicast(void* smem_dst, const void* gsrc, uint32_t bytes, uint64_t* bar, uint16_t mask) {
-  asm volatile("cp.async.bulk.shared::cluster.global.mbarrier::complete_tx::bytes.multicast::cluster [%0], [%1], %2, [%3], %4;\n"
-               ::"r"(smem_u32(smem_dst)), "l"(gsrc), "r"(bytes), "r"(smem_u32(bar)), "h"(mask) : "memory");
+__device__ __forceinline__ uint32_t cluster_map(const void* p, uint32_t rank) {
+  uint32_t r;
+  asm volatile("mapa.shared::cluster.u32 %0, %1, %2;\n" : "=r"(r) : "r"(smem_u32(p)), "r"(rank));
+  return r;
+}
+__device__ __forceinline__ float ld_cluster_f32(uint32_t addr) {
+  float v;
+  asm volatile("ld.shared::cluster.f32 %0, [%1];\n" : "=f"(v) : "r"(addr));
+  return v;
+}
+__device__ __forceinline__ void mbar_arrive_cluster(uint64_t* bar, uint32_t rank) {
+  asm volatile("mbarrier.arrive.release.cluster.shared::cluster.b64 _, [%0];\n" ::"r"(cluster_map(bar, rank)) : "memory");
+}
+__device__ __forceinline__ void mbar_wait_cluster(uint64_t* bar, uint32_t parity) {
+  const uint32_t addr = smem_u32(bar);
+  uint32_t done = 0;
+#pragma unroll 1
+  for (uint32_t it = 0; it < 20000000u; ++it) {
+    asm volatile("{\n .reg .pred p;\n mbarrier.try_wait.parity.acquire.cluster.shared::cta.b64 p, [%1], %2;\n selp.u32 %0, 1, 0, p;\n}\n"
+                 : "=r"(done) : "r"(addr), "r"(parity) : "memory");
+    if (done) return;
+  }
+  __trap();
 }
 __device__ __forceinline__ void fence_proxy_async() { asm volatile("fence.proxy.async;\n" ::: "memory"); }
 
```
